# LiangZhaoPKUImperial/LinearSFM

Hardware: AMD Instinct MI355X
Metric: hierarchical linear map-joining solve wall-clock, NC3500-like stereo (all transforms + joins) (lower is better)
Workload: dtype f64

## Files before the change

include/lsfm.h:

```cpp
#ifndef LSFM_H
#define LSFM_H

#include <stddef.h>

#ifdef __cplusplus
extern "C" {
#endif

#define LSFM_OK 0
#define LSFM_ERR_ARG (-1)
#define LSFM_ERR_NO_DEVICE (-2)
#define LSFM_ERR_HIP (-3)
#define LSFM_ERR_OOM (-4)
#define LSFM_ERR_INTERNAL (-5)
#define LSFM_ERR_IO (-6)
#define LSFM_ERR_NOT_SPD (-7)
#define LSFM_NOT_CONVERGED 1

typedef struct lsfm_context lsfm_context;

typedef struct lsfm_map {
	int Ref, FRef, m, n, nU, nW;
	int ScaP, Fix, Sign, FScaP, FFix;
	int* stno;
// ... 176 lines not shown
int lsfm_read_pair_gate(const char* path, int* ids_f, int* ids_g, double* d2, double* cov_diff, int cap, int* count);
int lsfm_save_merge_report(const char* path, int K, int removed, int dof, double d2, const int* ids);
int lsfm_read_merge_report(const char* path, int* K, int* removed, int* dof, double* d2, int* ids, int cap);
int lsfm_save_pair_list(const char* path, const int* ids, long long K);
int lsfm_read_pair_list(const char* path, int* ids, long long cap, long long* count);
int lsfm_save_state(const char* path, const double* st, const int* stno, int n);
int lsfm_save_state_bin(const char* path, const double* st, const int* stno, int n);
int lsfm_save_poses(const char* pose_path, const char* feat_path, const int* stno, const double* st, int n);

int lsfm_spmv_bench(lsfm_context* ctx, int m, const int* rowptr, const int* colidx, const double* val,
                    const double* x, double* y, int reps, double* avg_ms, double* algorithmic_bytes);

int lsfm_wstream_bench(lsfm_context* ctx, long long nblocks, int mode, int reps, double* avg_ms);

int lsfm_selftest_prims(lsfm_context* ctx, int cases, unsigned seed);

int lsfm_selftest_vinv(lsfm_context* ctx, const double* V, const double* eb, int n, int skip, double* IV, double* LY);

#define LSFM_SELFTEST_CHOL_INFO 16
int lsfm_selftest_chol(lsfm_context* ctx, int m, const int* rowptr, const int* colidx, const double* val, const int* origin, const unsigned char* fixed,
                       const int* pose_seg, int nseg, const double* r, int nrhs, int mode, double* z, double* dot, int* perm, int* colptr, int* rowidx,
                       double* L, double* Dinv, double* dscale, int cap_blocks, int* info);

int lsfm_selftest_transform(lsfm_context* ctx, const lsfm_map* maps, int N, int mono, const int* tref, const int* tscap, const int* tfix,
                            int alias_passthrough, lsfm_map* out);

int lsfm_selftest_small(lsfm_context* ctx, int G, const int* pose_off, const int* feat_off, const int* u_off, const unsigned char* active,
                        const double* U, const int* Ui, const int* Uj, const double* W, const int* photo, const int* feature, int nW, const double* V,
                        const double* ea, const double* eb, const double* x0, const unsigned char* fixed, int strips, double* x_pose, double* x_feat,
                        int* status, double* max_rel);
// ... 6 lines not shown
```

linearsfm_amd/api.py:

```python
from __future__ import annotations

import ctypes as C
import os

import numpy as np

_HERE = os.path.dirname(os.path.abspath(__file__))
LIB_PATH = os.path.join(_HERE, "liblsfm_hip.so")
_LIB = None

LSFM_OK = 0
LSFM_NOT_CONVERGED = 1


class LsfmMap(C.Structure):
    _fields_ = [("Ref", C.c_int), ("FRef", C.c_int), ("m", C.c_int), ("n", C.c_int), ("nU", C.c_int), ("nW", C.c_int),
                ("ScaP", C.c_int), ("Fix", C.c_int), ("Sign", C.c_int), ("FScaP", C.c_int), ("FFix", C.c_int),
                ("stno", C.POINTER(C.c_int)), ("stVal", C.POINTER(C.c_double)),
                ("U", C.POINTER(C.c_double)), ("Ui", C.POINTER(C.c_int)), ("Uj", C.POINTER(C.c_int)),
                ("W", C.POINTER(C.c_double)), ("photo", C.POINTER(C.c_int)), ("feature", C.POINTER(C.c_int)),
                ("V", C.POINTER(C.c_double)), ("FBlock", C.POINTER(C.c_int)), ("pose_origin", C.POINTER(C.c_int))]


class LsfmStats(C.Structure):
# ... 119 lines not shown
        L.lsfm_read_pair_gate.argtypes = [C.c_char_p, ip, ip, dp, dp, C.c_int, ip]
        L.lsfm_map_marginalise.argtypes = [vp, P(LsfmMap), P(C.c_ubyte), P(LsfmMap)]
        L.lsfm_map_marginalise_timed.argtypes = [vp, P(LsfmMap), P(C.c_ubyte), P(LsfmMap), dp]
        ub = P(C.c_ubyte)
        L.lsfm_map_marginalise_poses.argtypes = [vp, P(LsfmMap), C.c_int, ub, ub, P(LsfmMap)]
        L.lsfm_map_marginalise_poses_timed.argtypes = [vp, P(LsfmMap), C.c_int, ub, ub, P(LsfmMap), dp, ip]
        L.lsfm_marg_pose_structure.argtypes = [P(LsfmMap), C.c_int, ub, ub, ub, ip, ip, ip, C.c_int, ip, ip, ip, C.c_int, ip, C.c_char_p, C.c_int]
        L.lsfm_gn_structure.argtypes = [P(LsfmMap), C.c_int, C.c_int, P(LsfmMap), C.c_int, C.c_int, ip, ip, ip, ip, ip, C.c_int, ip, ip, C.c_int, ip, ip, ip,
                                        C.c_int, ip, ip, C.c_int, ip, ip, ip, ip, C.c_int, C.c_char_p, C.c_int]
        L.lsfm_tree_export_reduced_size.argtypes = [vp, vp, ip, C.c_int, P(C.c_size_t)]
        L.lsfm_tree_export_reduced_dev.argtypes = [vp, vp, ip, C.c_int, vp, C.c_size_t]
        L.lsfm_tree_export_reduced_dev_timed.argtypes = [vp, vp, ip, C.c_int, vp, C.c_size_t, dp]
        L.lsfm_spmv_bench.argtypes = [vp, C.c_int, ip, ip, dp, dp, dp, C.c_int, dp, dp]
        L.lsfm_wstream_bench.argtypes = [vp, C.c_longlong, C.c_int, C.c_int, dp]
        L.lsfm_selftest_prims.argtypes = [vp, C.c_int, C.c_uint]
        L.lsfm_selftest_chol.argtypes = [vp, C.c_int, ip, ip, dp, ip, P(C.c_ubyte), ip, C.c_int, dp, C.c_int, C.c_int, dp, dp, ip, ip, ip, dp, dp, dp,
                                         C.c_int, ip]
        L.lsfm_selftest_transform.argtypes = [vp, P(LsfmMap), C.c_int, C.c_int, ip, ip, ip, C.c_int, P(LsfmMap)]
        L.lsfm_selftest_small.argtypes = [vp, C.c_int, ip, ip, ip, ub, dp, ip, ip, dp, ip, ip, C.c_int, dp, dp, dp, dp, ub, C.c_int, dp, dp, ip, dp]
        _LIB = L
    return _LIB


EXPORTS = ["lsfm_context_create", "lsfm_context_destroy", "lsfm_set_pcg", "lsfm_set_precision", "lsfm_set_small_solve", "lsfm_set_spmv_variant", "lsfm_set_covcols_panel", "lsfm_last_error", "lsfm_stream",
           "lsfm_map_release", "lsfm_transform_stereo", "lsfm_transform_mono", "lsfm_join_stereo", "lsfm_join_mono",
           "lsfm_solve_stereo", "lsfm_solve_mono", "lsfm_tree_upload", "lsfm_tree_run", "lsfm_tree_set_final_reanchor",
           "lsfm_tree_download", "lsfm_tree_set_stop_level", "lsfm_tree_node_count", "lsfm_tree_download_node", "lsfm_tree_download_state", "lsfm_tree_set_plans", "lsfm_tree_export_size", "lsfm_tree_export_dev", "lsfm_packed_size",
           "lsfm_tree_upload_dev", "lsfm_tree_reload_dev", "lsfm_tree_set_comm", "lsfm_tree_set_comm_blocks", "lsfm_tree_export_slice_sizes", "lsfm_tree_export_slice_dev",
           "lsfm_tree_free", "lsfm_divide_conquer", "lsfm_read_localmap", "lsfm_read_localmaps", "lsfm_write_localmap", "lsfm_write_mapset", "lsfm_mapset_info", "lsfm_mapset_stamp", "lsfm_read_mapset", "lsfm_save_state_bin", "lsfm_save_state", "lsfm_save_poses", "lsfm_gn_polish",
           "lsfm_gn_polish_robust", "lsfm_map_chi2", "lsfm_map_feature_chi2", "lsfm_gn_polish_robust_features", "lsfm_gn_linearise", "lsfm_gn_linearise_timed",
           "lsfm_spmv_bench", "lsfm_wstream_bench", "lsfm_selftest_prims", "lsfm_selftest_chol", "lsfm_selftest_transform", "lsfm_selftest_small", "lsfm_schur_pattern", "lsfm_symbolic_analyse", "lsfm_inverse_v", "lsfm_selftest_vinv", "lsfm_solve_features",
           "lsfm_map_covariance", "lsfm_map_covariance_timed",
           "lsfm_save_covariances", "lsfm_read_covariances",
           "lsfm_map_covariance_columns", "lsfm_map_covariance_columns_timed", "lsfm_save_cov_columns", "lsfm_read_cov_columns",
           "lsfm_map_covariance_feature_columns", "lsfm_map_covariance_feature_columns_timed", "lsfm_map_feature_pair_gate", "lsfm_map_feature_pair_gate_timed", "lsfm_save_pair_gate", "lsfm_read_pair_gate",
           "lsfm_map_merge_features", "lsfm_map_merge_features_timed", "lsfm_merge_structure", "lsfm_save_merge_report", "lsfm_read_merge_report",
           "lsfm_map_feature_pair_candidates", "lsfm_map_feature_pair_candidates_timed", "lsfm_save_pair_list", "lsfm_read_pair_list",
           "lsfm_map_marginalise", "lsfm_map_marginalise_timed", "lsfm_tree_export_reduced_size", "lsfm_tree_export_reduced_dev",
           "lsfm_tree_export_reduced_dev_timed", "lsfm_map_marginalise_poses", "lsfm_map_marginalise_poses_timed", "lsfm_marg_pose_structure", "lsfm_gn_structure"]


def _c(a, dtype):
    return np.ascontiguousarray(a, dtype=dtype).reshape(-1)


def _ptr(a, ctype):
    return a.ctypes.data_as(C.POINTER(ctype))


class HostMap:

    def __init__(self, d):
        g = d if isinstance(d, dict) else d.__dict__
        self.stno = _c(g["stno"], np.int32); self.stVal = _c(g["stVal"], np.float64)
# ... 545 lines not shown
        y = np.zeros(6 * m)
        ms, by = C.c_double(), C.c_double()
        self._check(lib().lsfm_spmv_bench(self._h, m, _ptr(rowptr, C.c_int), _ptr(colidx, C.c_int), _ptr(val, C.c_double),
                                          _ptr(x, C.c_double), _ptr(y, C.c_double), int(reps), C.byref(ms), C.byref(by)),
                    "lsfm_spmv_bench")
        return y, ms.value, by.value


def _wstream(self, nblocks, mode, reps=10):
    ms = C.c_double()
    self._check(lib().lsfm_wstream_bench(self._h, int(nblocks), int(mode), int(reps), C.byref(ms)), "lsfm_wstream_bench")
    return ms.value


Context.wstream_bench = _wstream


def _selftest_prims(self, cases=64, seed=1):
    self._check(lib().lsfm_selftest_prims(self._h, int(cases), int(seed)), "lsfm_selftest_prims")


Context.selftest_prims = _selftest_prims

SELFTEST_CHOL_INFO = ("blocks", "leaf_tasks", "leaf_columns", "task0_outer", "groups", "group_levels", "fused_levels", "split_levels", "max_rows_below",
                      "d_err", "floored")


def _selftest_chol(self, rowptr, colidx, val, r, origin=None, fixed=None, pose_seg=None, nseg=1, mode=0):
    rowptr = _c(rowptr, np.int32); colidx = _c(colidx, np.int32); val = _c(val, np.float64)
    m = len(rowptr) - 1
# ... 352 lines not shown
```

linearsfm_amd/csrc/lsfm_internal.hpp:

```cpp
#pragma once
#include <hip/hip_runtime.h>

#include <cstdint>
#include <cstdio>
#include <condition_variable>
#include <cstring>
#include <exception>
#include <functional>
#include <memory>
#include <mutex>
#include <thread>
#include <string>
#include <vector>

#include "../../include/lsfm.h"
#include "lsfm_map.hpp"

namespace lsfm {

struct Error { int code; std::string msg; };
struct DevBatch;
struct IndexHold;
struct SolvePlan;
struct PreLevel;
// ... 48 lines not shown
	double* W = nullptr; int *photo = nullptr, *feature = nullptr;
	int* fptr = nullptr;
	double* V = nullptr;
	const double* W_alias = nullptr;
	const int* d_alias = nullptr;
	const unsigned long long* s_keys = nullptr;
	int s_nnzb = 0;
};

struct PcgOptions { double rel_tol = 1e-12; int max_steps = 50; bool mixed = false; int spmv_variant = 0; };

struct LevelIndex {
	int NU = -1, NW = -1, NF = -1;
	const int *KU = nullptr, *KW = nullptr;
	const int *match = nullptr, *R = nullptr;
	std::shared_ptr<IndexHold> own;
};
const int* level_index_keep(lsfm_context* ctx, LevelIndex& li, const int* src, size_t n);

struct LevelPlan {
	bool valid = false;
	LevelIndex idx;
	std::vector<int> tr_cnt;
	std::vector<int> tr_sign;
	std::vector<int> join_rb;
	std::vector<int> join_uo, join_wo;
	std::shared_ptr<SolvePlan> solve;
};

struct RunStatsDev {
// ... 337 lines not shown
```

linearsfm_amd/csrc/lsfm_join.hip:

```cpp
#include "lsfm_device.hpp"
#include "lsfm_internal.hpp"
#include <climits>
#include "lsfm_join.hpp"
#include "lsfm_solve.hpp"

namespace lsfm {

__device__ __forceinline__ unsigned long long jh_mix(unsigned long long x)
{
	x ^= x >> 33; x *= 0xff51afd7ed558ccdull; x ^= x >> 33; x *= 0xc4ceb9fe1a85ec53ull; x ^= x >> 33;
	return x;
}
__global__ void k_join_hash_insert(int NF, const int* __restrict__ feat_id, const int* __restrict__ feat_map, unsigned long long* tab,
                                   int* __restrict__ tval, unsigned long long mask)
{
	int f = blockIdx.x * blockDim.x + threadIdx.x;
	if (f >= NF) return;
	const int mp = feat_map[f];
	if (mp & 1) return;
	const unsigned long long key = ((unsigned long long)(mp >> 1) << 32) | (unsigned)feat_id[f];
	unsigned long long h = jh_mix(key) & mask;
	for (;;)
	{
		const unsigned long long old = atomicCAS(&tab[h], ~0ull, key);
// ... 42 lines not shown
	jr.match = ctx->scratch.alloc<int>(in.NF + 1);
	int* unm = ctx->scratch.alloc<int>(in.NF + 2);
	jr.R = ctx->scratch.alloc<int>(in.NF + 2);
	if (in.NF) join_match_features(ctx, in, jr.match, unm);
	else dev_zero(ctx, unm, 2 * sizeof(int));
	dev_exclusive_scan(ctx, unm, jr.R, in.NF);
	return jr;
}

__global__ void k_gather_at(const int* __restrict__ src, const int* __restrict__ idx, int n, int* __restrict__ out)
{
	int i = blockIdx.x * blockDim.x + threadIdx.x;
	if (i < n) out[i] = src[idx[i]];
}

__global__ void k_join_features(int NF, const int* __restrict__ feat_map, const int* __restrict__ feat_id, const double* __restrict__ feat,
                                const double* __restrict__ V, const int* __restrict__ fptr, const int* __restrict__ match,
                                const int* __restrict__ R, const JGroup* __restrict__ grp, int* __restrict__ newf, int* __restrict__ lenE,
                                int* __restrict__ lenC, double* __restrict__ Vy, double* __restrict__ eF, int* __restrict__ fid_y,
                                double* __restrict__ feat_y, int* __restrict__ srcE, int* __restrict__ srcC, int side)
{
	int f = blockIdx.x * blockDim.x + threadIdx.x;
	if (f >= NF) return;
	int mp = feat_map[f];
	const JGroup& g = grp[mp >> 1];
	int nf;
	const bool cur = mp & 1;
	if ((int)cur != side) return;
	if (!cur) nf = g.FY0 + (f - g.F0E);
	else if (match[f] >= 0) nf = g.FY0 + (match[f] - g.F0E);
	else nf = g.FY0 + g.nE + (R[f] - g.rC0);
	newf[f] = nf;
	const bool first = !cur || match[f] < 0;
	int len = fptr[f + 1] - fptr[f];
	if (!cur) { lenE[nf] = len; lenC[nf] = 0; }
	else { lenC[nf] = len; if (first) lenE[nf] = 0; }
	if (srcE)
	{
		if (!cur) { srcE[nf] = f; srcC[nf] = -1; }
		else { srcC[nf] = f; if (first) srcE[nf] = -1; }
	}
	const double* v = V + (size_t)f * 9;
	const double* x = feat + (size_t)f * 3;
	if (first)
	{
		for (int i = 0; i < 9; i++) Vy[(size_t)nf * 9 + i] = v[i];
		for (int r = 0; r < 3; r++) eF[(size_t)nf * 3 + r] = v[3 * r] * x[0] + v[3 * r + 1] * x[1] + v[3 * r + 2] * x[2];
	}
	else
	{
		for (int i = 0; i < 9; i++) Vy[(size_t)nf * 9 + i] += v[i];
		for (int r = 0; r < 3; r++) eF[(size_t)nf * 3 + r] += v[3 * r] * x[0] + v[3 * r + 1] * x[1] + v[3 * r + 2] * x[2];
	}
	if (first)
	{
		fid_y[nf] = feat_id[f];
		feat_y[(size_t)nf * 3] = x[0]; feat_y[(size_t)nf * 3 + 1] = x[1]; feat_y[(size_t)nf * 3 + 2] = x[2];
	}
}

__global__ void k_add_lens(int n, const int* __restrict__ a, const int* __restrict__ b, int* __restrict__ out)
{
	int i = blockIdx.x * blockDim.x + threadIdx.x;
	if (i < n) out[i] = a[i] + b[i];
	if (i == 0) out[n] = 0;
}

__global__ void k_join_wbase(int NF, const int* __restrict__ feat_map, const int* __restrict__ newf, const int* __restrict__ lenE,
                             const int* __restrict__ fptr_y, int* __restrict__ wbase)
{
	int f = blockIdx.x * blockDim.x + threadIdx.x;
	if (f >= NF) return;
	const int nf = newf[f];
// ... 105 lines not shown
	io.ea = eP; io.eb = eF; io.d_pose_origin = out.pose_origin;
	io.x_pose = out.pose; io.x_feat = out.feat;
	io.seg_rows = seg_rows;
	io.index_arrays_at_evA = at_evA; io.step_hint = step_hint;
	small_level_offsets(ctx, out, io);
	return io;
}

void join_close(lsfm_context* ctx, size_t smark, const SolveOutcome& oc, bool whole_level)
{
	ctx->scratch.release(smark);
	if (oc.not_converged > 0 && ctx->stats) ctx->stats->not_converged += oc.not_converged;
	if (ctx->plan && whole_level) ctx->plan->valid = true;
}

void join_stereo_prepare(lsfm_context* ctx, Arena& ar, const DevBatch& in, DevBatch& out, JoinState& st, const DevBatch* level_in, const int* hub)
{
	hipStream_t s = ctx->stream;
	const int B = in.B, G = (B + 1) / 2;
	st.smark = ctx->scratch.mark();

	LevelPlan* plan = ctx->plan;
	const int *match = nullptr, *R = nullptr;
	const int nb = (in.NF + 255) / 256;
	std::vector<int> rb(B + 1);
	if (ctx->warm() && plan->idx.match && plan->idx.R && plan->idx.NF == in.NF)
	{
		match = plan->idx.match; R = plan->idx.R;
		rb = plan->join_rb;
	}
// ... 46 lines not shown
	out.pose_id = ar.alloc<int>(in.M);
	out.pose_origin = ar.alloc<int>(in.M);
	cb.d2d(out.pose_origin, in.pose_origin, (size_t)in.M * sizeof(int));
	out.feat = ar.alloc<double>((size_t)NFY * 3);
	out.feat_id = ar.alloc<int>(NFY);
	out.U = ar.alloc<double>((size_t)in.NU * 36); out.Ui = ar.alloc<int>(in.NU); out.Uj = ar.alloc<int>(in.NU);
	out.W = ar.alloc<double>((size_t)in.NW * 18); out.photo = ar.alloc<int>(in.NW); out.feature = ar.alloc<int>(in.NW);
	out.fptr = ar.alloc<int>(NFY + 1);
	out.V = ar.alloc<double>((size_t)NFY * 9);
	batch_set_offsets(ctx, ar, out, &cb);
	cb.d2d(out.pose_id, in.pose_id, (size_t)in.M * sizeof(int));
	st.d_act = reinterpret_cast<unsigned char*>(ctx->scratch.alloc<int>((G + 3) / 4 + 1));
	st.act_padded.assign(((size_t)G + 3) / 4 * 4, 0);
	std::copy(seg_active.begin(), seg_active.end(), st.act_padded.begin());
	cb.h2d(st.d_act, st.act_padded.data(), st.act_padded.size());
	cb.flush();
	batch_fill_maps(ctx, out);
	int* newf = st.newf = ctx->scratch.alloc<int>(in.NF + 1);
	int* lens = ctx->scratch.alloc<int>(NFY + 2);
	st.srcf = ctx->scratch.alloc<int>(in.NW + 1);
	int* lenE = st.lenE = ctx->scratch.alloc<int>(NFY + 1);
	int* lenC = ctx->scratch.alloc<int>(NFY + 1);
	double* eF = st.eF = ctx->scratch.alloc<double>((size_t)NFY * 3);
	double* eP = st.eP = ctx->scratch.alloc<double>((size_t)in.M * 6);
	dev_zero(ctx, eP, (size_t)in.M * 6 * sizeof(double));
	const bool small_level = small_level_strips(ctx, seg_rows) > 0;
	const bool early = !small_level && !ctx->comm && !(ctx->pre && !ctx->pre_plan.valid) && level_in && hub && !ctx->warm() && level_in->NF == in.NF && level_in->M == in.M;
	st.fuse_rhs = !small_level && !ctx->comm && !ctx->pcg.mixed;
	int *srcE = nullptr, *srcC = nullptr;
	if (early || st.fuse_rhs)
	{
		srcE = ctx->scratch.alloc<int>(NFY + 1); srcC = ctx->scratch.alloc<int>(NFY + 1);
	}
	st.srcE = srcE; st.srcC = srcC;
	if (in.NF)
		for (int side = 0; side < 2; side++)
			hipLaunchKernelGGL(k_join_features, dim3(nb), dim3(256), 0, s, in.NF, in.feat_map, in.feat_id, in.feat, in.V, in.fptr, match, R, d_grp,
			                   newf, lenE, lenC, out.V, eF, out.feat_id, out.feat, srcE, srcC, side);
	if (early)
	{
		const DevBatch& X = *level_in;
		EarlyPatternIn ei;
		ei.M = in.M; ei.NFY = NFY; ei.NU = X.NU;
		ei.Ui = X.Ui; ei.Uj = X.Uj; ei.pose_map = X.pose_map; ei.hub = hub;
		ei.fptr = X.fptr; ei.photo = X.photo; ei.feat_map = X.feat_map; ei.srcE = srcE; ei.srcC = srcC;
		LSFM_CHECK_HIP(hipEventRecord(ctx->ord[evC_pairs], s));
		schur_pattern_early_issue(ctx, ei);
	}
	else schur_pattern_early_drop(ctx);
	hipLaunchKernelGGL(k_add_lens, dim3((NFY + 256) / 256), dim3(256), 0, s, NFY, lenE, lenC, lens);
	dev_exclusive_scan(ctx, lens, out.fptr, NFY);
	if (early) LSFM_CHECK_HIP(hipEventRecord(ctx->ord[evC_runs], s));
	st.wbase = ctx->scratch.alloc<int>(in.NF + 1);
	if (in.NF) hipLaunchKernelGGL(k_join_wbase, dim3(nb), dim3(256), 0, s, in.NF, in.feat_map, newf, lenE, out.fptr, st.wbase);
	LSFM_CHECK_HIP(hipGetLastError());
	ctx->mark("jn_prep");
}

SolveOutcome join_stereo_finish(lsfm_context* ctx, const DevBatch& in, DevBatch& out, JoinState& st, double* eP_out, double* eF_out, int step_hint)
{
	hipStream_t s = ctx->stream;
	const int NFY = out.NF;
	double *eP = st.eP, *eF = st.eF;
	int* srcf = st.srcf;
	if (in.NU)
	{
		CopyBatch cu(ctx);
		cu.d2d(out.U, in.U, (size_t)in.NU * 36 * sizeof(double));
		cu.d2d(out.Ui, in.Ui, (size_t)in.NU * sizeof(int));
		cu.d2d(out.Uj, in.Uj, (size_t)in.NU * sizeof(int));
// ... 41 lines not shown
```

linearsfm_amd/csrc/lsfm_join.hpp:

```cpp
#pragma once
#include "lsfm_internal.hpp"

namespace lsfm {

struct JGroup {
	int F0E, nE, F0C, nC;
	int FY0;
	int rC0;
};

struct JoinState {
	size_t smark = 0;
	int *newf = nullptr, *lenE = nullptr, *srcf = nullptr, *wbase = nullptr;
	double *eP = nullptr, *eF = nullptr;
	std::vector<unsigned char> seg_active, act_padded;
	unsigned char* d_act = nullptr;
	std::vector<int> seg_rows;
	bool fuse_rhs = false;
	int *srcE = nullptr, *srcC = nullptr;
};
void join_stereo_prepare(lsfm_context* ctx, Arena& ar, const DevBatch& in, DevBatch& out, JoinState& st, const DevBatch* level_in, const int* hub);
SolveOutcome join_stereo_finish(lsfm_context* ctx, const DevBatch& in, DevBatch& out, JoinState& st, double* eP_out, double* eF_out, int step_hint = 0);

void join_match_features(lsfm_context* ctx, const DevBatch& in, int* match, int* unm);
struct JoinRanks { int *match, *R; };
JoinRanks join_rank_features(lsfm_context* ctx, const DevBatch& in);
void join_layout(int B, const std::vector<int>& feat_off, const std::vector<int>& pose_off, const std::vector<int>& rb, int shared, DevBatch& out,
                 std::vector<JGroup>& grp, std::vector<int>& seg_rows, std::vector<unsigned char>& seg_active);
SolveIO join_solve_io(lsfm_context* ctx, const DevBatch& out, const unsigned char* d_act, const double* eP, const double* eF,
                      const std::vector<int>& seg_rows, bool at_evA, int step_hint);
void join_close(lsfm_context* ctx, size_t smark, const SolveOutcome& oc, bool whole_level);
__global__ void k_gather_at(const int* __restrict__ src, const int* __restrict__ idx, int n, int* __restrict__ out);
__global__ void k_join_features(int NF, const int* __restrict__ feat_map, const int* __restrict__ feat_id, const double* __restrict__ feat,
                                const double* __restrict__ V, const int* __restrict__ fptr, const int* __restrict__ match,
                                const int* __restrict__ R, const JGroup* __restrict__ grp, int* __restrict__ newf, int* __restrict__ lenE,
// ... 5 lines not shown
```

linearsfm_amd/csrc/lsfm_level.hip:

```cpp
#include <algorithm>
#include <chrono>
#include <cmath>
#include <cstdlib>

#include "lsfm_device.hpp"
#include "lsfm_symbolic.hpp"
#include "lsfm_pcg.hpp"

namespace lsfm {

struct SolvePlan {
	SchurSystem sy;
	CholDev ch;
	int its = 1;
	bool mixed = false;
	double rel_tol = 0;
	bool small = false;
	char* mem = nullptr;
	~SolvePlan() { if (mem) (void)hipFree(mem); }
};
static std::shared_ptr<SolvePlan> solve_plan_store(lsfm_context* ctx, const SchurSystem& sy, const CholDev& ch, int its)
{
	auto sp = std::make_shared<SolvePlan>();
	const size_t M = sy.M, nnzb = sy.nnzb, cap = (size_t)sy.mask + 1;
// ... 70 lines not shown
	pl->M = Y.M;
	Arena& sa = ctx->sarena[next_level & 1];
	sa.reset();
	std::vector<int> counts;
	LevelIndex kept;
	bool ok = false;
	{
		Fork side(ctx, ctx->stream3, evY, false, &sa);
		if (ctx->timeline_on) { (void)hipEventSynchronize(ctx->ord[evY]); ctx->mark("pre_evY"); }
		int* d_tref = ctx->scratch.alloc<int>(Y.B);
		h2d(ctx, d_tref, target_ref.data(), sizeof(int) * (size_t)Y.B);
		ok = schur_pattern_prefetch(ctx, Y, d_tref, level_keys, level_nnzb, pl->sy, whole ? &counts : nullptr, !next_small, whole ? &kept : nullptr);
		if (ok)
		{
			if (!next_small) chol_fetch(ctx, pl->sy, Y.pose_origin, pl->hin);
			side.done(evP);
		}
	}
	ctx->mark("pre_pat");
	if (!ok) return;
	if (!next_small)
	{
		if (!ctx->worker) ctx->worker.reset(new HostWorker());
		PreLevel* raw = pl.get();
		ctx->worker->run([raw]() { chol_symbolic(raw->hin.keys.data(), raw->sy.nnzb, raw->hin.origin.data(), raw->sy.M, raw->sym); });
		pl->worker = ctx->worker.get();
		ctx->mark("pre_sym");
		pl->whole = whole; pl->level = next_level; pl->its = step_hint;
		ctx->pre = pl;
	}
// ... 59 lines not shown
__global__ void k_digest_compare(const unsigned long long* d, int* mismatch)
{
	if (d[0] != d[1]) atomicAdd(mismatch, 1);
}
__global__ void k_chol_err_to_run(const int* err, RunStatsDev* run)
{
	if (*err && !run->chol_err) run->chol_err = *err;
}

struct LevelStructure {
	SchurSystem sy;
	CholDev ch;
	SolvePlan* sp = nullptr;
	double tw0 = 0, tw1 = 0;
};
static double wall_ms() { return std::chrono::duration<double, std::milli>(std::chrono::steady_clock::now().time_since_epoch()).count(); }
static LevelStructure level_structure(lsfm_context* ctx, const SolveIO& io, SolvePlan* sp, PreLevel* pre, bool pending, hipEvent_t eb)
{
	hipStream_t s = ctx->stream;
	LevelStructure ls;
	SchurSystem& sy = ls.sy;
	CholDev& ch = ls.ch;
	auto assemble = [&]() {
		build_schur_values(ctx, io, sy);
		LSFM_REC_T(eb, s); if (roctx().mark) roctx().mark("lsfm factor + refine: begin");
	};
	if (sp || pending)
	{
		sy = pending ? pre->sy : sp->sy;
		schur_vinv(ctx, io, sy);
		assemble();
		if (pending)
		{
			ctx->mark("k9_enq");
			ctx->plan->solve = pre_plan_complete(ctx, *pre);
			sp = ctx->plan->solve.get();
			ctx->mark("sym_wait");
		}
		ls.sp = sp;
		ch = sp->ch;
		chol_alloc_values(ctx, ch);
		return ls;
	}
	schur_vinv(ctx, io, sy);
// ... 247 lines not shown
```

linearsfm_amd/csrc/lsfm_pattern.hip:

```cpp
#include <algorithm>

#include "lsfm_device.hpp"
#include "lsfm_internal.hpp"
#include "lsfm_join.hpp"
#include "lsfm_solve.hpp"

namespace lsfm {

__global__ void k_fill_u64(unsigned long long* p, size_t n, unsigned long long v)
{
	size_t i = (size_t)blockIdx.x * blockDim.x + threadIdx.x;
	if (i < n) p[i] = v;
}

__global__ void k_pat_insert_keys(int n, const unsigned long long* __restrict__ keys, unsigned long long* tab, unsigned long long mask, int* overflow)
{
	int i = blockIdx.x * blockDim.x + threadIdx.x;
	if (i < n) hash_insert(tab, mask, keys[i], overflow);
}

__global__ void k_pat_insert_u(int NU, int M, const int* __restrict__ Ui, const int* __restrict__ Uj, const int* __restrict__ pose_map,
                               const int* __restrict__ hub, unsigned long long* tab, unsigned long long mask, int* overflow)
{
	int i = blockIdx.x * blockDim.x + threadIdx.x;
// ... 412 lines not shown
		hipLaunchKernelGGL(k_pre_flags, dim3((nmax + 255) / 256), dim3(256), 0, s, Y.Ui, Y.Uj, Y.NU, Y.photo, Y.NW, Y.pose_map, hub, keepU, keepW);
		dev_exclusive_scan(ctx, keepU, KU, Y.NU);
		dev_exclusive_scan(ctx, keepW, KW, Y.NW);
		dev_exclusive_scan(ctx, unm, R, Y.NF);
		int* d_off = sc.alloc<int>(2 * (B + 1));
		h2d(ctx, d_off, Y.u_off.data(), (B + 1) * sizeof(int));
		h2d(ctx, d_off + B + 1, Y.w_off.data(), (B + 1) * sizeof(int));
		int* d_cnt = sc.alloc<int>(3 * (B + 1));
		hipLaunchKernelGGL(k_pre_gather, dim3((B + 1 + 127) / 128), dim3(128), 0, s, KU, KW, R, d_off, d_off + B + 1, Y.d_feat_off, B, d_cnt);
		counts->resize(3 * (size_t)(B + 1));
		LSFM_CHECK_HIP(hipMemcpyAsync(counts->data(), d_cnt, counts->size() * sizeof(int), hipMemcpyDeviceToHost, s));
		if (keep)
		{
			*keep = LevelIndex();
			keep->NU = Y.NU; keep->NW = Y.NW; keep->NF = Y.NF;
			keep->KU = KU; keep->KW = KW; keep->match = match; keep->R = R;
		}
	}
	if (!want_pattern)
	{
		LSFM_CHECK_HIP(hipStreamSynchronize(s));
		return true;
	}
	return pattern_build(ctx, Y.M, pattern_capacity(std::max((size_t)Y.NU + Y.M, (size_t)prev_nnzb + Y.M), Y.M), sy, [&](const PatternBuild& pb) {
		const int nu = std::max(Y.NU, Y.M);
		hipLaunchKernelGGL(k_pat_insert_u, dim3((nu + 255) / 256), dim3(256), 0, s, Y.NU, Y.M, Y.Ui, Y.Uj, Y.pose_map, hub, pb.tab, pb.mask(), pb.d_flags);
		if (prev_keys && prev_nnzb) hipLaunchKernelGGL(k_pat_insert_keys, dim3((prev_nnzb + 255) / 256), dim3(256), 0, s, prev_nnzb, prev_keys, pb.tab, pb.mask(), pb.d_flags);
		if (!prev_keys) pat_insert_w(s, Y.NF, Y.fptr, Y.photo, pb);
		if (Y.NF)
		{
			PatPairsIn in;
// ... 8 lines not shown
```

Before: 30.05.

## Precompute next-level join structure and Schur slot tables one level ahead

During the level-ahead prepare step, the joined-map feature structure (newf, wbase, lenE, srcE/srcC, fid_y, fptr_y) and the K9 Schur slot tables are now built early. The join and solve then take these precomputed arrays instead of recomputing them, using a new values-only join kernel. On warm runs the structure saved from the cold run is reused. The goal is to take structural index work off the critical path of each join and Schur assembly, at the cost of extra scratch memory, more kernels in the prepare phase, and a correctness risk if the cached structure goes stale (an env-gated check is provided).

```diff
diff --git a/include/lsfm.h b/include/lsfm.h
--- a/include/lsfm.h
+++ b/include/lsfm.h
@@ -214,6 +214,7 @@
 int lsfm_wstream_bench(lsfm_context* ctx, long long nblocks, int mode, int reps, double* avg_ms);
 
 int lsfm_selftest_prims(lsfm_context* ctx, int cases, unsigned seed);
+void lsfm_debug_struct_ahead(int* out, int reset);
 
 int lsfm_selftest_vinv(lsfm_context* ctx, const double* V, const double* eb, int n, int skip, double* IV, double* LY);
 
diff --git a/linearsfm_amd/api.py b/linearsfm_amd/api.py
--- a/linearsfm_amd/api.py
+++ b/linearsfm_amd/api.py
@@ -157,6 +157,8 @@
         L.lsfm_spmv_bench.argtypes = [vp, C.c_int, ip, ip, dp, dp, dp, C.c_int, dp, dp]
         L.lsfm_wstream_bench.argtypes = [vp, C.c_longlong, C.c_int, C.c_int, dp]
         L.lsfm_selftest_prims.argtypes = [vp, C.c_int, C.c_uint]
+        L.lsfm_debug_struct_ahead.argtypes = [ip, C.c_int]
+        L.lsfm_debug_struct_ahead.restype = None
         L.lsfm_selftest_chol.argtypes = [vp, C.c_int, ip, ip, dp, ip, P(C.c_ubyte), ip, C.c_int, dp, C.c_int, C.c_int, dp, dp, ip, ip, ip, dp, dp, dp,
                                          C.c_int, ip]
         L.lsfm_selftest_transform.argtypes = [vp, P(LsfmMap), C.c_int, C.c_int, ip, ip, ip, C.c_int, P(LsfmMap)]
@@ -180,7 +182,8 @@
            "lsfm_map_merge_features", "lsfm_map_merge_features_timed", "lsfm_merge_structure", "lsfm_save_merge_report", "lsfm_read_merge_report",
            "lsfm_map_feature_pair_candidates", "lsfm_map_feature_pair_candidates_timed", "lsfm_save_pair_list", "lsfm_read_pair_list",
            "lsfm_map_marginalise", "lsfm_map_marginalise_timed", "lsfm_tree_export_reduced_size", "lsfm_tree_export_reduced_dev",
-           "lsfm_tree_export_reduced_dev_timed", "lsfm_map_marginalise_poses", "lsfm_map_marginalise_poses_timed", "lsfm_marg_pose_structure", "lsfm_gn_structure"]
+           "lsfm_tree_export_reduced_dev_timed", "lsfm_map_marginalise_poses", "lsfm_map_marginalise_poses_timed", "lsfm_marg_pose_structure", "lsfm_gn_structure",
+           "lsfm_debug_struct_ahead"]
 
 
 def _c(a, dtype):
@@ -756,6 +759,12 @@
 
 
 Context.wstream_bench = _wstream
+
+
+def struct_ahead_counts(reset=False):
+    out = np.zeros(3, np.int32)
+    lib().lsfm_debug_struct_ahead(_ptr(out, C.c_int), int(bool(reset)))
+    return int(out[0]), int(out[1]), int(out[2])
 
 
 def _selftest_prims(self, cases=64, seed=1):
diff --git a/linearsfm_amd/csrc/lsfm_internal.hpp b/linearsfm_amd/csrc/lsfm_internal.hpp
--- a/linearsfm_amd/csrc/lsfm_internal.hpp
+++ b/linearsfm_amd/csrc/lsfm_internal.hpp
@@ -86,6 +86,14 @@
 	int NU = -1, NW = -1, NF = -1;
 	const int *KU = nullptr, *KW = nullptr;
 	const int *match = nullptr, *R = nullptr;
+	int NFt = -1, NWt = -1, NFY = -1;
+	const int *newf = nullptr, *wbase = nullptr;
+	const int *lenE = nullptr, *srcE = nullptr, *srcC = nullptr, *fid_y = nullptr;
+	const int* fptr_y = nullptr;
+	const int *hub = nullptr, *photo_y = nullptr;
+	int *k9_ns = nullptr, *k9_pose = nullptr, *k9_wlist = nullptr, *k9_wcnt = nullptr;
+	unsigned char* k9_eslot = nullptr;
+	int k9_tiles = 0;
 	std::shared_ptr<IndexHold> own;
 };
 const int* level_index_keep(lsfm_context* ctx, LevelIndex& li, const int* src, size_t n);
diff --git a/linearsfm_amd/csrc/lsfm_join.hip b/linearsfm_amd/csrc/lsfm_join.hip
--- a/linearsfm_amd/csrc/lsfm_join.hip
+++ b/linearsfm_amd/csrc/lsfm_join.hip
@@ -80,19 +80,16 @@
 	if (i < n) out[i] = src[idx[i]];
 }
 
-__global__ void k_join_features(int NF, const int* __restrict__ feat_map, const int* __restrict__ feat_id, const double* __restrict__ feat,
-                                const double* __restrict__ V, const int* __restrict__ fptr, const int* __restrict__ match,
-                                const int* __restrict__ R, const JGroup* __restrict__ grp, int* __restrict__ newf, int* __restrict__ lenE,
-                                int* __restrict__ lenC, double* __restrict__ Vy, double* __restrict__ eF, int* __restrict__ fid_y,
-                                double* __restrict__ feat_y, int* __restrict__ srcE, int* __restrict__ srcC, int side)
-{
-	int f = blockIdx.x * blockDim.x + threadIdx.x;
-	if (f >= NF) return;
+__device__ __forceinline__ int join_feature_structure(int f, int side, const int* __restrict__ feat_map, const int* __restrict__ fptr,
+                                                      const int* __restrict__ match, const int* __restrict__ R, const JGroup* __restrict__ grp,
+                                                      int* __restrict__ newf, int* __restrict__ lenE, int* __restrict__ lenC,
+                                                      int* __restrict__ srcE, int* __restrict__ srcC, bool* first_out)
+{
 	int mp = feat_map[f];
 	const JGroup& g = grp[mp >> 1];
 	int nf;
 	const bool cur = mp & 1;
-	if ((int)cur != side) return;
+	if ((int)cur != side) return -1;
 	if (!cur) nf = g.FY0 + (f - g.F0E);
 	else if (match[f] >= 0) nf = g.FY0 + (match[f] - g.F0E);
 	else nf = g.FY0 + g.nE + (R[f] - g.rC0);
@@ -106,6 +103,21 @@
 		if (!cur) { srcE[nf] = f; srcC[nf] = -1; }
 		else { srcC[nf] = f; if (first) srcE[nf] = -1; }
 	}
+	*first_out = first;
+	return nf;
+}
+
+__global__ void k_join_features(int NF, const int* __restrict__ feat_map, const int* __restrict__ feat_id, const double* __restrict__ feat,
+                                const double* __restrict__ V, const int* __restrict__ fptr, const int* __restrict__ match,
+                                const int* __restrict__ R, const JGroup* __restrict__ grp, int* __restrict__ newf, int* __restrict__ lenE,
+                                int* __restrict__ lenC, double* __restrict__ Vy, double* __restrict__ eF, int* __restrict__ fid_y,
+                                double* __restrict__ feat_y, int* __restrict__ srcE, int* __restrict__ srcC, int side)
+{
+	int f = blockIdx.x * blockDim.x + threadIdx.x;
+	if (f >= NF) return;
+	bool first;
+	const int nf = join_feature_structure(f, side, feat_map, fptr, match, R, grp, newf, lenE, lenC, srcE, srcC, &first);
+	if (nf < 0) return;
 	const double* v = V + (size_t)f * 9;
 	const double* x = feat + (size_t)f * 3;
 	if (first)
@@ -123,6 +135,40 @@
 		fid_y[nf] = feat_id[f];
 		feat_y[(size_t)nf * 3] = x[0]; feat_y[(size_t)nf * 3 + 1] = x[1]; feat_y[(size_t)nf * 3 + 2] = x[2];
 	}
+}
+__global__ void k_join_structure(int NF, const int* __restrict__ feat_map, const int* __restrict__ feat_id, const int* __restrict__ fptr,
+                                 const int* __restrict__ match, const int* __restrict__ R, const JGroup* __restrict__ grp, int* __restrict__ newf,
+                                 int* __restrict__ lenE, int* __restrict__ lenC, int* __restrict__ fid_y, int* __restrict__ srcE, int* __restrict__ srcC, int side)
+{
+	int f = blockIdx.x * blockDim.x + threadIdx.x;
+	if (f >= NF) return;
+	bool first;
+	const int nf = join_feature_structure(f, side, feat_map, fptr, match, R, grp, newf, lenE, lenC, srcE, srcC, &first);
+	if (nf >= 0 && first) fid_y[nf] = feat_id[f];
+}
+__global__ void k_join_values(int NFY, const int* __restrict__ srcE, const int* __restrict__ srcC, const double* __restrict__ feat,
+                              const double* __restrict__ V, double* __restrict__ Vy, double* __restrict__ eF, double* __restrict__ feat_y)
+{
+	int nf = blockIdx.x * blockDim.x + threadIdx.x;
+	if (nf >= NFY) return;
+	const int e = srcE[nf], c = srcC[nf];
+	const int f1 = e >= 0 ? e : c;
+	if (f1 < 0) return;
+	const double* v = V + (size_t)f1 * 9;
+	const double* x = feat + (size_t)f1 * 3;
+	double vy[9], ef[3];
+	for (int i = 0; i < 9; i++) vy[i] = v[i];
+	for (int r = 0; r < 3; r++) ef[r] = v[3 * r] * x[0] + v[3 * r + 1] * x[1] + v[3 * r + 2] * x[2];
+	feat_y[(size_t)nf * 3] = x[0]; feat_y[(size_t)nf * 3 + 1] = x[1]; feat_y[(size_t)nf * 3 + 2] = x[2];
+	if (e >= 0 && c >= 0)
+	{
+		const double* v2 = V + (size_t)c * 9;
+		const double* x2 = feat + (size_t)c * 3;
+		for (int i = 0; i < 9; i++) vy[i] += v2[i];
+		for (int r = 0; r < 3; r++) ef[r] += v2[3 * r] * x2[0] + v2[3 * r + 1] * x2[1] + v2[3 * r + 2] * x2[2];
+	}
+	for (int i = 0; i < 9; i++) Vy[(size_t)nf * 9 + i] = vy[i];
+	for (int r = 0; r < 3; r++) eF[(size_t)nf * 3 + r] = ef[r];
 }
 
 __global__ void k_add_lens(int n, const int* __restrict__ a, const int* __restrict__ b, int* __restrict__ out)
@@ -258,6 +304,144 @@
 	if (ctx->plan && whole_level) ctx->plan->valid = true;
 }
 
+bool struct_ahead_enabled()
+{
+	static const bool off = getenv("LSFM_NO_STRUCT_AHEAD") != nullptr;
+	return !off;
+}
+static int g_struct_joins[3];
+int& struct_ahead_k9_levels() { return g_struct_joins[2]; }
+extern "C" void lsfm_debug_struct_ahead(int* out, int reset)
+{
+	if (out) { out[0] = g_struct_joins[0]; out[1] = g_struct_joins[1]; out[2] = g_struct_joins[2]; }
+	if (reset) g_struct_joins[0] = g_struct_joins[1] = g_struct_joins[2] = 0;
+}
+
+struct PreMap { int active, F0, W0, W0n, kW0, pad; };
+__global__ void k_join_pre_fptr(int NF, const int* __restrict__ feat_map, const int* __restrict__ fptr, const int* __restrict__ KW,
+                                const PreMap* __restrict__ pm, int NWt, int* __restrict__ nfptr)
+{
+	int f = blockIdx.x * blockDim.x + threadIdx.x;
+	if (f == 0) nfptr[NF] = NWt;
+	if (f >= NF) return;
+	const PreMap t = pm[feat_map[f]];
+	const int j0 = fptr[f];
+	nfptr[f] = t.active ? t.W0n + (f - t.F0) + (KW[j0] - t.kW0) : t.W0n + (j0 - t.W0);
+}
+
+__global__ void k_join_pre_photo(int NF, int NW, const int* __restrict__ feat_map, const int* __restrict__ fptr, const int* __restrict__ feature,
+                                 const int* __restrict__ photo, const int* __restrict__ KW, const PreMap* __restrict__ pm, const int* __restrict__ hub,
+                                 const int* __restrict__ wbase, int* __restrict__ photo_y)
+{
+	int i = blockIdx.x * blockDim.x + threadIdx.x;
+	if (i < NF)
+	{
+		const int b = feat_map[i];
+		if (pm[b].active) photo_y[wbase[i]] = hub[b];
+	}
+	if (i >= NW) return;
+	const int f = feature[i], j0 = fptr[f];
+	if (!pm[feat_map[f]].active) photo_y[wbase[f] + (i - j0)] = photo[i];
+	else if (KW[i + 1] - KW[i]) photo_y[wbase[f] + 1 + (KW[i] - KW[j0])] = photo[i];
+}
+
+static void join_run_pointers(lsfm_context* ctx, int NF, int NFY, const int* feat_map, const int* newf, const int* lenE, const int* lenC, int* lens,
+                              int* fptr_y, int* wbase)
+{
+	hipStream_t s = ctx->stream;
+	hipLaunchKernelGGL(k_add_lens, dim3((NFY + 256) / 256), dim3(256), 0, s, NFY, lenE, lenC, lens);
+	dev_exclusive_scan(ctx, lens, fptr_y, NFY);
+	if (NF) hipLaunchKernelGGL(k_join_wbase, dim3((NF + 255) / 256), dim3(256), 0, s, NF, feat_map, newf, lenE, fptr_y, wbase);
+}
+
+void join_structure_ahead(lsfm_context* ctx, const DevBatch& Y, const std::vector<int>& target_ref, const std::vector<int>& counts, LevelIndex& li)
+{
+	hipStream_t s = ctx->stream;
+	Arena& sc = ctx->scratch;
+	const int B = Y.B, G = (B + 1) / 2, NF = Y.NF;
+	if (!NF || !li.KW || !li.match || !li.R || li.NF != NF || counts.size() != 3 * (size_t)(B + 1)) return;
+	std::vector<PreMap> pm(B);
+	int W0n = 0;
+	for (int b = 0; b < B; b++)
+	{
+		PreMap& t = pm[b];
+		t.active = target_ref[b] >= 0 && !map_in_frame(Y, b, target_ref[b], 0, false);
+		t.F0 = Y.feat_off[b]; t.W0 = Y.w_off[b]; t.W0n = W0n; t.kW0 = counts[B + 1 + b]; t.pad = 0;
+		W0n += (t.active ? Y.feat_off[b + 1] - t.F0 : 0) + counts[B + 1 + b + 1] - counts[B + 1 + b];
+	}
+	const int NWt = W0n;
+	const std::vector<int> rb(counts.begin() + 2 * (B + 1), counts.end());
+	DevBatch lay;
+	std::vector<JGroup> grp;
+	std::vector<int> seg_rows;
+	std::vector<unsigned char> seg_active;
+	join_layout(B, Y.feat_off, Y.pose_off, rb, 0, lay, grp, seg_rows, seg_active);
+	const int NFY = lay.feat_off[G];
+	PreMap* d_pm = sc.alloc<PreMap>(B);
+	JGroup* d_grp = sc.alloc<JGroup>(G);
+	h2d(ctx, d_pm, pm.data(), sizeof(PreMap) * B);
+	h2d(ctx, d_grp, grp.data(), sizeof(JGroup) * G);
+	int* nfptr = sc.alloc<int>(NF + 1);
+	int* newf = sc.alloc<int>(NF + 1); int* wbase = sc.alloc<int>(NF + 1);
+	int* lenE = sc.alloc<int>(NFY + 1); int* lenC = sc.alloc<int>(NFY + 1); int* lens = sc.alloc<int>(NFY + 2);
+	int* srcE = sc.alloc<int>(NFY + 1); int* srcC = sc.alloc<int>(NFY + 1); int* fid_y = sc.alloc<int>(NFY + 1);
+	int* fptr_y = sc.alloc<int>(NFY + 1);
+	const int nb = (NF + 255) / 256;
+	hipLaunchKernelGGL(k_join_pre_fptr, dim3(nb), dim3(256), 0, s, NF, Y.feat_map, Y.fptr, li.KW, d_pm, NWt, nfptr);
+	for (int side = 0; side < 2; side++)
+		hipLaunchKernelGGL(k_join_structure, dim3(nb), dim3(256), 0, s, NF, Y.feat_map, Y.feat_id, nfptr, li.match, li.R, d_grp, newf, lenE, lenC, fid_y,
+		                   srcE, srcC, side);
+	join_run_pointers(ctx, NF, NFY, Y.feat_map, newf, lenE, lenC, lens, fptr_y, wbase);
+	LSFM_CHECK_HIP(hipGetLastError());
+	li.NFt = NF; li.NWt = NWt; li.NFY = NFY;
+	li.newf = newf; li.wbase = wbase; li.lenE = lenE; li.srcE = srcE; li.srcC = srcC; li.fid_y = fid_y; li.fptr_y = fptr_y;
+	if (!li.hub || li.NW != Y.NW) return;
+	int* photo_y = sc.alloc<int>(NWt + 1);
+	const int nmax = std::max(NF, Y.NW);
+	hipLaunchKernelGGL(k_join_pre_photo, dim3((nmax + 255) / 256), dim3(256), 0, s, NF, Y.NW, Y.feat_map, Y.fptr, Y.feature, Y.photo, li.KW, d_pm, li.hub,
+	                   wbase, photo_y);
+	const int ntiles = (NFY + LSFM_PM_TILE - 1) / LSFM_PM_TILE;
+	K9Cache kc;
+	kc.ns = sc.alloc<int>(ntiles + 1);
+	kc.pose = sc.alloc<int>((size_t)ntiles * 64 + 1);
+	kc.eslot = sc.alloc<unsigned char>((size_t)NWt + 1);
+	kc.wlist = sc.alloc<int>((size_t)3 * ntiles + 1);
+	kc.wcnt = sc.alloc<int>(8);
+	unsigned char* fb = sc.alloc<unsigned char>(ntiles + 1);
+	launch_schur_slots(ctx, NFY, fptr_y, photo_y, fb, kc);
+	LSFM_CHECK_HIP(hipGetLastError());
+	li.photo_y = photo_y;
+	li.k9_ns = kc.ns; li.k9_pose = kc.pose; li.k9_eslot = kc.eslot; li.k9_wlist = kc.wlist; li.k9_wcnt = kc.wcnt; li.k9_tiles = ntiles;
+}
+
+static void join_structure_check(lsfm_context* ctx, const DevBatch& in, int NFY, const JGroup* d_grp, const int* match, const int* R, const LevelIndex& li)
+{
+	Arena& sc = ctx->scratch;
+	const size_t mk = sc.mark();
+	const int NF = in.NF, nb = (NF + 255) / 256;
+	int* newf = sc.alloc<int>(NF + 1); int* wbase = sc.alloc<int>(NF + 1);
+	int* lenE = sc.alloc<int>(NFY + 1); int* lenC = sc.alloc<int>(NFY + 1); int* lens = sc.alloc<int>(NFY + 2);
+	int* srcE = sc.alloc<int>(NFY + 1); int* srcC = sc.alloc<int>(NFY + 1); int* fid_y = sc.alloc<int>(NFY + 1);
+	int* fptr_y = sc.alloc<int>(NFY + 1);
+	for (int side = 0; side < 2; side++)
+		hipLaunchKernelGGL(k_join_structure, dim3(nb), dim3(256), 0, ctx->stream, NF, in.feat_map, in.feat_id, in.fptr, match, R, d_grp, newf, lenE, lenC,
+		                   fid_y, srcE, srcC, side);
+	join_run_pointers(ctx, NF, NFY, in.feat_map, newf, lenE, lenC, lens, fptr_y, wbase);
+	auto same = [&](const char* what, const int* a, const int* b, size_t n) {
+		std::vector<int> ha(n), hb(n);
+		d2h(ctx, ha.data(), a, n * sizeof(int));
+		d2h(ctx, hb.data(), b, n * sizeof(int));
+		for (size_t i = 0; i < n; i++)
+			if (ha[i] != hb[i])
+				LSFM_FAIL(LSFM_ERR_INTERNAL, std::string("joint-map structure taken from the plan: ") + what + "[" + std::to_string(i) + "] is " + std::to_string(ha[i]) +
+				                                 ", the join's own kernels give " + std::to_string(hb[i]));
+	};
+	same("newf", li.newf, newf, NF); same("wbase", li.wbase, wbase, NF);
+	same("lenE", li.lenE, lenE, NFY); same("fid_y", li.fid_y, fid_y, NFY); same("fptr_y", li.fptr_y, fptr_y, (size_t)NFY + 1);
+	same("srcE", li.srcE, srcE, NFY); same("srcC", li.srcC, srcC, NFY);
+	sc.release(mk);
+}
+
 void join_stereo_prepare(lsfm_context* ctx, Arena& ar, const DevBatch& in, DevBatch& out, JoinState& st, const DevBatch* level_in, const int* hub)
 {
 	hipStream_t s = ctx->stream;
@@ -334,19 +518,43 @@
 	st.act_padded.assign(((size_t)G + 3) / 4 * 4, 0);
 	std::copy(seg_active.begin(), seg_active.end(), st.act_padded.begin());
 	cb.h2d(st.d_act, st.act_padded.data(), st.act_padded.size());
+	const bool small_level = small_level_strips(ctx, seg_rows) > 0;
+	st.fuse_rhs = !small_level && !ctx->comm && !ctx->pcg.mixed;
+	const LevelIndex* pi = (struct_ahead_enabled() && ctx->warm() && !ctx->comm && !small_level && match == plan->idx.match) ? &plan->idx : nullptr;
+	const bool ahead = pi && pi->newf && in.NF > 0 && pi->NFt == in.NF && pi->NWt == in.NW && pi->NFY == NFY && pi->srcE && pi->srcC;
+	if (ctx->in_tree_run && level_in && !small_level) g_struct_joins[ahead ? 0 : 1]++;
+	if (ahead)
+	{
+		cb.d2d(out.fptr, pi->fptr_y, ((size_t)NFY + 1) * sizeof(int));
+		cb.d2d(out.feat_id, pi->fid_y, (size_t)NFY * sizeof(int));
+	}
 	cb.flush();
 	batch_fill_maps(ctx, out);
-	int* newf = st.newf = ctx->scratch.alloc<int>(in.NF + 1);
+	if (ahead)
+	{
+		if (getenv("LSFM_CHECK_STRUCT_AHEAD")) join_structure_check(ctx, in, NFY, d_grp, match, R, *pi);
+		st.newf = pi->newf; st.lenE = pi->lenE; st.wbase = pi->wbase; st.srcE = pi->srcE; st.srcC = pi->srcC;
+		st.srcf = ctx->scratch.alloc<int>(in.NW + 1);
+		st.eF = ctx->scratch.alloc<double>((size_t)NFY * 3);
+		st.eP = ctx->scratch.alloc<double>((size_t)in.M * 6);
+		dev_zero(ctx, st.eP, (size_t)in.M * 6 * sizeof(double));
+		hipLaunchKernelGGL(k_join_values, dim3((NFY + 255) / 256), dim3(256), 0, s, NFY, pi->srcE, pi->srcC, in.feat, in.V, out.V, st.eF, out.feat);
+		schur_pattern_early_drop(ctx);
+		LSFM_CHECK_HIP(hipGetLastError());
+		ctx->mark("jn_prep");
+		return;
+	}
+	int* newf = ctx->scratch.alloc<int>(in.NF + 1);
+	st.newf = newf;
 	int* lens = ctx->scratch.alloc<int>(NFY + 2);
 	st.srcf = ctx->scratch.alloc<int>(in.NW + 1);
-	int* lenE = st.lenE = ctx->scratch.alloc<int>(NFY + 1);
+	int* lenE = ctx->scratch.alloc<int>(NFY + 1);
+	st.lenE = lenE;
 	int* lenC = ctx->scratch.alloc<int>(NFY + 1);
 	double* eF = st.eF = ctx->scratch.alloc<double>((size_t)NFY * 3);
 	double* eP = st.eP = ctx->scratch.alloc<double>((size_t)in.M * 6);
 	dev_zero(ctx, eP, (size_t)in.M * 6 * sizeof(double));
-	const bool small_level = small_level_strips(ctx, seg_rows) > 0;
 	const bool early = !small_level && !ctx->comm && !(ctx->pre && !ctx->pre_plan.valid) && level_in && hub && !ctx->warm() && level_in->NF == in.NF && level_in->M == in.M;
-	st.fuse_rhs = !small_level && !ctx->comm && !ctx->pcg.mixed;
 	int *srcE = nullptr, *srcC = nullptr;
 	if (early || st.fuse_rhs)
 	{
@@ -371,9 +579,22 @@
 	hipLaunchKernelGGL(k_add_lens, dim3((NFY + 256) / 256), dim3(256), 0, s, NFY, lenE, lenC, lens);
 	dev_exclusive_scan(ctx, lens, out.fptr, NFY);
 	if (early) LSFM_CHECK_HIP(hipEventRecord(ctx->ord[evC_runs], s));
-	st.wbase = ctx->scratch.alloc<int>(in.NF + 1);
-	if (in.NF) hipLaunchKernelGGL(k_join_wbase, dim3(nb), dim3(256), 0, s, in.NF, in.feat_map, newf, lenE, out.fptr, st.wbase);
+	int* wbase = ctx->scratch.alloc<int>(in.NF + 1);
+	st.wbase = wbase;
+	if (in.NF) hipLaunchKernelGGL(k_join_wbase, dim3(nb), dim3(256), 0, s, in.NF, in.feat_map, newf, lenE, out.fptr, wbase);
 	LSFM_CHECK_HIP(hipGetLastError());
+	if (struct_ahead_enabled() && plan && !ctx->warm() && plan != &ctx->pre_plan && ctx->in_tree_run && !ctx->comm && !small_level && in.NF && srcE)
+	{
+		LevelIndex& li = plan->idx;
+		li.newf = level_index_keep(ctx, li, newf, (size_t)in.NF + 1);
+		li.wbase = level_index_keep(ctx, li, wbase, (size_t)in.NF + 1);
+		li.lenE = level_index_keep(ctx, li, lenE, (size_t)NFY + 1);
+		li.srcE = level_index_keep(ctx, li, srcE, (size_t)NFY + 1);
+		li.srcC = level_index_keep(ctx, li, srcC, (size_t)NFY + 1);
+		li.fid_y = level_index_keep(ctx, li, out.feat_id, (size_t)NFY);
+		li.fptr_y = level_index_keep(ctx, li, out.fptr, (size_t)NFY + 1);
+		li.NFt = in.NF; li.NWt = in.NW; li.NFY = NFY;
+	}
 	ctx->mark("jn_prep");
 }
 
diff --git a/linearsfm_amd/csrc/lsfm_join.hpp b/linearsfm_amd/csrc/lsfm_join.hpp
--- a/linearsfm_amd/csrc/lsfm_join.hpp
+++ b/linearsfm_amd/csrc/lsfm_join.hpp
@@ -11,14 +11,18 @@
 
 struct JoinState {
 	size_t smark = 0;
-	int *newf = nullptr, *lenE = nullptr, *srcf = nullptr, *wbase = nullptr;
+	const int *newf = nullptr, *lenE = nullptr, *wbase = nullptr;
+	int* srcf = nullptr;
 	double *eP = nullptr, *eF = nullptr;
 	std::vector<unsigned char> seg_active, act_padded;
 	unsigned char* d_act = nullptr;
 	std::vector<int> seg_rows;
 	bool fuse_rhs = false;
-	int *srcE = nullptr, *srcC = nullptr;
+	const int *srcE = nullptr, *srcC = nullptr;
 };
+void join_structure_ahead(lsfm_context* ctx, const DevBatch& Y, const std::vector<int>& target_ref, const std::vector<int>& counts, LevelIndex& li);
+bool struct_ahead_enabled();
+int& struct_ahead_k9_levels();
 void join_stereo_prepare(lsfm_context* ctx, Arena& ar, const DevBatch& in, DevBatch& out, JoinState& st, const DevBatch* level_in, const int* hub);
 SolveOutcome join_stereo_finish(lsfm_context* ctx, const DevBatch& in, DevBatch& out, JoinState& st, double* eP_out, double* eF_out, int step_hint = 0);
 
diff --git a/linearsfm_amd/csrc/lsfm_level.hip b/linearsfm_amd/csrc/lsfm_level.hip
--- a/linearsfm_amd/csrc/lsfm_level.hip
+++ b/linearsfm_amd/csrc/lsfm_level.hip
@@ -4,6 +4,7 @@
 #include <cstdlib>
 
 #include "lsfm_device.hpp"
+#include "lsfm_join.hpp"
 #include "lsfm_symbolic.hpp"
 #include "lsfm_pcg.hpp"
 
@@ -108,6 +109,7 @@
 		if (ok)
 		{
 			if (!next_small) chol_fetch(ctx, pl->sy, Y.pose_origin, pl->hin);
+			if (whole && !next_small && struct_ahead_enabled()) join_structure_ahead(ctx, Y, target_ref, counts, kept);
 			side.done(evP);
 		}
 	}
@@ -197,6 +199,60 @@
 	SolvePlan* sp = nullptr;
 	double tw0 = 0, tw1 = 0;
 };
+static void prepared_k9_check(lsfm_context* ctx, const SolveIO& io, const LevelIndex& li)
+{
+	Arena& sc = ctx->scratch;
+	const size_t mk = sc.mark();
+	const int nt = li.k9_tiles, NW = io.NW;
+	K9Cache kc;
+	kc.ns = sc.alloc<int>(nt + 1); kc.pose = sc.alloc<int>((size_t)nt * 64 + 1); kc.eslot = sc.alloc<unsigned char>((size_t)NW + 1);
+	kc.wlist = sc.alloc<int>((size_t)3 * nt + 1); kc.wcnt = sc.alloc<int>(8);
+	unsigned char* fb = sc.alloc<unsigned char>(nt + 1);
+	launch_schur_slots(ctx, io.NF, io.fptr, io.photo, fb, kc);
+	auto fail = [](const std::string& what, size_t i, long a, long b) {
+		LSFM_FAIL(LSFM_ERR_INTERNAL, "prepared one level ahead: " + what + "[" + std::to_string(i) + "] is " + std::to_string(a) + ", the level's own kernels give " + std::to_string(b));
+	};
+	auto ints = [&](const int* d, size_t n) { std::vector<int> h(n); d2h(ctx, h.data(), d, n * sizeof(int)); return h; };
+	auto bytes = [&](const unsigned char* d, size_t n) { std::vector<unsigned char> h(n); d2h(ctx, h.data(), d, n); return h; };
+	const std::vector<int> pa = ints(li.photo_y, NW), pb = ints(io.photo, NW), fp = ints(io.fptr, (size_t)io.NF + 1);
+	for (int j = 0; j < NW; j++) if (pa[j] != pb[j]) fail("photo", j, pa[j], pb[j]);
+	const std::vector<int> na = ints(li.k9_ns, nt), nb = ints(kc.ns, nt), qa = ints(li.k9_pose, (size_t)nt * 64), qb = ints(kc.pose, (size_t)nt * 64);
+	const std::vector<unsigned char> ea = bytes(li.k9_eslot, NW), eb = bytes(kc.eslot, NW);
+	for (int t = 0; t < nt; t++)
+	{
+		if (na[t] != nb[t]) fail("K9 ns", t, na[t], nb[t]);
+		if (na[t] == -1000) continue;
+		const size_t q0 = (size_t)t * 64;
+		const int n = std::min(std::abs(na[t]), 64);
+		std::vector<int> sa(qa.begin() + q0, qa.begin() + q0 + n), sb(qb.begin() + q0, qb.begin() + q0 + n);
+		std::sort(sa.begin(), sa.end()); std::sort(sb.begin(), sb.end());
+		for (int q = 0; q < n; q++) if (sa[q] != sb[q]) fail("K9 pose (sorted, of tile " + std::to_string(t) + ")", q, sa[q], sb[q]);
+		for (int j = fp[(size_t)t * LSFM_PM_TILE]; j < fp[std::min((size_t)(t + 1) * LSFM_PM_TILE, (size_t)io.NF)]; j++)
+		{
+			if ((ea[j] & 0x80) != (eb[j] & 0x80)) fail("K9 eslot (repeat mark)", j, ea[j], eb[j]);
+			const int s = ea[j] & 0x7f;
+			if (s >= n || qa[q0 + s] != pb[j]) fail("pose of the K9 slot of block", j, s < n ? qa[q0 + s] : -1, pb[j]);
+		}
+	}
+	const std::vector<int> ca = ints(li.k9_wcnt, 3), cb = ints(kc.wcnt, 3), wa = ints(li.k9_wlist, (size_t)3 * nt), wb = ints(kc.wlist, (size_t)3 * nt);
+	for (int v = 0; v < 3; v++)
+	{
+		if (ca[v] != cb[v]) fail("K9 wcnt", v, ca[v], cb[v]);
+		for (int q = 0; q < ca[v]; q++)
+			if (wa[(size_t)v * nt + q] != wb[(size_t)v * nt + q]) fail("K9 wlist", (size_t)v * nt + q, wa[(size_t)v * nt + q], wb[(size_t)v * nt + q]);
+	}
+	sc.release(mk);
+}
+static void take_prepared_k9(lsfm_context* ctx, const SolveIO& io, SchurSystem& sy)
+{
+	const LevelIndex& li = ctx->pre_plan.idx;
+	if (!struct_ahead_enabled() || !li.k9_ns || !io.NF || li.NFY != io.NF || li.NWt != io.NW || li.k9_tiles != (io.NF + LSFM_PM_TILE - 1) / LSFM_PM_TILE) return;
+	if (getenv("LSFM_CHECK_STRUCT_AHEAD")) prepared_k9_check(ctx, io, li);
+	sy.k9.ns = li.k9_ns; sy.k9.pose = li.k9_pose; sy.k9.eslot = li.k9_eslot; sy.k9.wlist = li.k9_wlist; sy.k9.wcnt = li.k9_wcnt;
+	sy.k9_tiles = li.k9_tiles; sy.k9_NW = io.NW;
+	struct_ahead_k9_levels()++;
+}
+
 static double wall_ms() { return std::chrono::duration<double, std::milli>(std::chrono::steady_clock::now().time_since_epoch()).count(); }
 static LevelStructure level_structure(lsfm_context* ctx, const SolveIO& io, SolvePlan* sp, PreLevel* pre, bool pending, hipEvent_t eb)
 {
@@ -211,6 +267,7 @@
 	if (sp || pending)
 	{
 		sy = pending ? pre->sy : sp->sy;
+		if (pending) take_prepared_k9(ctx, io, sy);
 		schur_vinv(ctx, io, sy);
 		assemble();
 		if (pending)
diff --git a/linearsfm_amd/csrc/lsfm_pattern.hip b/linearsfm_amd/csrc/lsfm_pattern.hip
--- a/linearsfm_amd/csrc/lsfm_pattern.hip
+++ b/linearsfm_amd/csrc/lsfm_pattern.hip
@@ -450,7 +450,7 @@
 		{
 			*keep = LevelIndex();
 			keep->NU = Y.NU; keep->NW = Y.NW; keep->NF = Y.NF;
-			keep->KU = KU; keep->KW = KW; keep->match = match; keep->R = R;
+			keep->KU = KU; keep->KW = KW; keep->match = match; keep->R = R; keep->hub = hub;
 		}
 	}
 	if (!want_pattern)
```

New measurement: 30.00, median of 5. Within noise of the previous version (-0.2%).
